# shayneobrien/generative-models

Measured on AMD Instinct MI355X. Metric: images/sec (28x28 MNIST) per D+G step, NSGAN bs=256, higher is better.
Workload: dtype f32; 1 GPU; NSGAN MNIST bs=256 fp32 per GPU (BASELINE.json configs[1]); 784-400-20 MLPs, N=50000 synthetic Bernoulli images, parity-mode RNG protocol, Adam 2e-4, D_steps=1; global_batch=256, parallelism=dp1, ranks_seen=1, gradient_exchange=none (1 rank), timing=one 2064-step timed region, cold_start_inclusive=False

## Files before the change

generative_models_amd/csrc/gm_gemm.hip:

```cpp
#include "gm_common.h"
#include "gm_head.h"
#include "gm_gather.h"
#include "gm_dvae.h"
#include "gm_ldsdma.h"

#include <cstdlib>
#include <type_traits>

typedef float f32x16 __attribute__((ext_vector_type(16)));

#ifdef GM_STAMPS
namespace gm_stamps {
constexpr int WAVES = 16, IDS = 40, HDR = 8, MAXB = 512, SLOT_WORDS = HDR + 2 * MAXB + WAVES * IDS * 2, SLOTS = 64;
static unsigned long long* host_buf = nullptr;
static int host_tile = 0, host_next = 0;
struct Ctx { unsigned long long* slot; int tile; };
__device__ __forceinline__ void rec(const Ctx& c, int tile, int id) {
    if (!c.slot || tile != c.tile || (threadIdx.x & 63)) return;
    __builtin_amdgcn_sched_barrier(0);
    unsigned long long* w = c.slot + HDR + 2 * MAXB + ((threadIdx.x >> 6) * IDS + id) * 2;
    w[0] = clock64(); w[1] = wall_clock64();
    __builtin_amdgcn_sched_barrier(0);
}
__device__ __forceinline__ void edge(const Ctx& c, bool exit_, int tile, int M, int N, int K, int mode) {
    if (!c.slot || threadIdx.x) return;
    const int blk = blockIdx.y * gridDim.x + blockIdx.x;
    if (blk < MAXB) c.slot[HDR + 2 * blk + (exit_ ? 1 : 0)] = wall_clock64();
    if (!exit_ && tile == 0) {
        c.slot[0] = 1; c.slot[2] = (unsigned long long)gridDim.x * gridDim.y; c.slot[3] = M; c.slot[4] = N; c.slot[5] = K;
        c.slot[6] = mode; c.slot[7] = blockDim.x;
    }
}
}
#define GM_STAMP(ctx, tile, id) gm_stamps::rec((ctx), (tile), (id))
#define GM_STAMP_EDGE(p, exit_, tile, mode) gm_stamps::edge((p).stamp, (exit_), (tile), (p).M, (p).N, (p).K, (mode))
#define GM_STAMP_AFTER(v) asm volatile("" ::"v"(v))
extern "C" int gm_stamps_set(unsigned long long* dev_buf, int probe_tile) {
    gm_stamps::host_buf = dev_buf; gm_stamps::host_tile = probe_tile; gm_stamps::host_next = 0;
    return 0;
}
extern "C" int gm_stamps_layout(int* out6) {
    out6[0] = gm_stamps::WAVES; out6[1] = gm_stamps::IDS; out6[2] = gm_stamps::HDR; out6[3] = gm_stamps::SLOT_WORDS;
    out6[4] = gm_stamps::SLOTS; out6[5] = gm_stamps::MAXB;
    return 0;
}
#else
#define GM_STAMP(slot, tile, id) do {} while (0)
#define GM_STAMP_EDGE(p, exit_, tile, mode) do {} while (0)
#define GM_STAMP_AFTER(v) do {} while (0)
#endif

namespace {

constexpr int TM = 32, TN = 32;

enum { MODE_FWD = 0, MODE_DX = 1, MODE_DW = 2 };

struct GemmP {
// ... 157 lines not shown
        }
    } else if (MODE == MODE_DX) {
        if (p.add) {
            const float4 a = ld4(p.add + (int64_t)m * p.ldadd + n);
            v.x += p.add_scale * a.x; v.y += p.add_scale * a.y; v.z += p.add_scale * a.z; v.w += p.add_scale * a.w;
        }
        if (p.epi == GM_ACT_RELU) {
            const float4 y = ld4(p.aux + (int64_t)m * p.ldaux + n);
            v.x = (y.x > 0.f) ? v.x : 0.f; v.y = (y.y > 0.f) ? v.y : 0.f; v.z = (y.z > 0.f) ? v.z : 0.f; v.w = (y.w > 0.f) ? v.w : 0.f;
        } else if (p.epi == GM_ACT_SIGMOID) {
            const float4 y = ld4(p.aux + (int64_t)m * p.ldaux + n);
            v.x = v.x * (y.x * (1.f - y.x)); v.y = v.y * (y.y * (1.f - y.y));
            v.z = v.z * (y.z * (1.f - y.z)); v.w = v.w * (y.w * (1.f - y.w));
        }
        float* cp = p.C + (int64_t)m * p.ldc + n;
        if (p.accumulate) { const float4 c = ld4(cp); v.x = c.x + v.x; v.y = c.y + v.y; v.z = c.z + v.z; v.w = c.w + v.w; }
        st4(cp, v);
    } else {
        const int64_t o = (int64_t)m * p.ldc + n;
        if (p.accumulate) { const float4 c = ld4(p.C + o); v.x += c.x; v.y += c.y; v.z += c.z; v.w += c.w; }
        st4(p.C + o, v);
        if (p.adam.enabled) {
            const int64_t si = gm_slot_index(p.adam.sched_slot);
            const float step_size = p.adam.sched[2 * si], bc2_sqrt = p.adam.sched[2 * si + 1];
            float4 P = ld4(p.adam.pW + o), M = ld4(p.adam.mW + o), V = ld4(p.adam.vW + o);
            adam_update(P.x, v.x, M.x, V.x, step_size, bc2_sqrt, p.adam.omb1, p.adam.b2, p.adam.omb2, p.adam.eps, p.adam.wd, p.adam.clamp);
            adam_update(P.y, v.y, M.y, V.y, step_size, bc2_sqrt, p.adam.omb1, p.adam.b2, p.adam.omb2, p.adam.eps, p.adam.wd, p.adam.clamp);
            adam_update(P.z, v.z, M.z, V.z, step_size, bc2_sqrt, p.adam.omb1, p.adam.b2, p.adam.omb2, p.adam.eps, p.adam.wd, p.adam.clamp);
            adam_update(P.w, v.w, M.w, V.w, step_size, bc2_sqrt, p.adam.omb1, p.adam.b2, p.adam.omb2, p.adam.eps, p.adam.wd, p.adam.clamp);
            st4(p.adam.pW + o, P); st4(p.adam.mW + o, M); st4(p.adam.vW + o, V);
        }
    }
}

template <int MODE>
__device__ __forceinline__ void store_group(const GemmP& p, float4 v, int m, int n, int ncap) {
    const int nreal = (MODE == MODE_DW) ? p.n_real : p.N;
    if (n + 3 < nreal && n + 3 < ncap) { store4<MODE>(p, v, m, n); return; }
    if (n < p.N && n < ncap) store_element<MODE>(p, v.x, m, n);
    if (n + 1 < p.N && n + 1 < ncap) store_element<MODE>(p, v.y, m, n + 1);
    if (n + 2 < p.N && n + 2 < ncap) store_element<MODE>(p, v.z, m, n + 2);
    if (n + 3 < p.N && n + 3 < ncap) store_element<MODE>(p, v.w, m, n + 3);
}

__device__ __forceinline__ int red_idx(int w, int row, int col) {
    return (w * 32 + row) * 32 + (col ^ ((((row >> 2) ^ row) & 1) << 4));
}

__device__ __forceinline__ int red_idx_sx(int w, int row, int col, int flip) {
    return (w * 32 + row) * 32 + (col ^ flip);
}

constexpr int KEEP_LD = 68;
template <int MODE, int WAVES, int ROWS = 32, bool LBL = false, int SXD = 0>
__device__ __forceinline__ void reduce_and_store(const GemmP& p, const float* red, int t, int m0,
                                                 int n0, int ncap = 0x7fffffff, int rcap = 32,
                                                 float* kept = nullptr, int srow0 = 0) {
    if (MODE == MODE_FWD && p.hd_part) {
#pragma unroll
        for (int e = 0; e < 1024 / (WAVES * 64); ++e) {
            const int row = (t >> 5) + e * (WAVES * 2), col = t & 31;
            const bool live = !(ROWS < 32 && row >= ROWS) && row < rcap;
            float v = 0.f;
            if (live) {
#pragma unroll
                for (int ww = 0; ww < WAVES; ++ww) v += red[red_idx(ww, row, col)];
            }
            const int m = m0 + row, n = n0 + col;
            const bool ok = live && m < p.M && n < p.N && n < ncap;
            float pv = 0.f;
            if (ok) {
                const float w = p.hd_w2[n];
                const float y = fwd_value(p, v, n);
                p.C[(int64_t)m * p.ldc + n] = y;
                pv = y * w;
                if (m == 0 && p.hd_snap) {
                    p.hd_snap[n] = w;
                    if (n == 0) p.hd_snap[p.N] = p.hd_b2[0];
                }
            }
#pragma unroll
            for (int o = 16; o > 0; o >>= 1) pv += __shfl_xor(pv, o, 64);
            if (col == 0 && live && m < p.M) p.hd_part[(int64_t)m * p.hd_ldp + (n0 >> 5)] = pv;
        }
        return;
    }
    if (MODE == MODE_FWD && p.sq_part) {
#pragma unroll
        for (int e = 0; e < 1024 / (WAVES * 64); ++e) {
            const int row = (t >> 5) + e * (WAVES * 2), col = t & 31;
            const bool live = !(ROWS < 32 && row >= ROWS) && row < rcap;
            float v = 0.f;
            if (live) {
#pragma unroll
                for (int ww = 0; ww < WAVES; ++ww) v += red[red_idx(ww, row, col)];
            }
            const int m = m0 + row, n = n0 + col;
            const bool ok = live && m < p.M && n < p.N && n < ncap;
            float pv = 0.f;
            if (ok) {
                const float r = fwd_value(p, v, n);
                p.C[(int64_t)m * p.ldc + n] = r;
                const float d = p.sq_x[(int64_t)m * p.sq_ldx + n] - r;
                pv = d * d;
                const float go = -(2.f * d);
                p.sq_dA[(int64_t)m * p.sq_lda + n] = (go * (1.f - r)) * r;
            }
#pragma unroll
            for (int o = 16; o > 0; o >>= 1) pv += __shfl_xor(pv, o, 64);
            if (col == 0 && live && m < p.M) p.sq_part[(int64_t)m * p.sq_ldp + (n0 >> 5)] = pv;
        }
        return;
    }
#pragma unroll
    for (int e = 0; e < 1024 / (WAVES * 64); ++e) {
        const int row = (t >> 5) + e * (WAVES * 2), col = t & 31;
        if ((ROWS < 32 && row >= ROWS) || row >= rcap) continue;
        float v = 0.f;
#pragma unroll
        for (int ww = 0; ww < WAVES; ++ww)
            v += red[SXD > 0 ? red_idx_sx(ww, row, col, ((srow0 + row) / (SXD > 0 ? SXD : 1)) & 1) : red_idx(ww, row, col)];
        const int m = m0 + row, n = n0 + col;
        if (m >= p.M || n >= p.N || n >= ncap) continue;
        store_element<MODE, LBL>(p, v, m, n, kept ? kept + row * KEEP_LD + col : nullptr);
    }
}

__device__ __forceinline__ float4 keep4(bool ok, float4 v) {
    return make_float4(ok ? v.x : 0.f, ok ? v.y : 0.f, ok ? v.z : 0.f, ok ? v.w : 0.f);
}

template <int NMFMA, int NDSR, int NVMEM, int NDSW>
__device__ __forceinline__ void lds_stage_schedule() {
    constexpr int NMEM = NDSR + NVMEM + NDSW;
    int done = 0;
#pragma unroll
    for (int q = 0; q < NMFMA; ++q) {
        __builtin_amdgcn_sched_group_barrier(0x008, 1, 0);
        const int upto = (NMEM * (q + 1) + NMFMA - 1) / NMFMA;
#pragma unroll
        for (int i = 0; i < 8; ++i) {
            if (done < upto) {
                if (done < NDSR) __builtin_amdgcn_sched_group_barrier(0x100, 1, 0);
                else if (done < NDSR + NVMEM) __builtin_amdgcn_sched_group_barrier(0x020, 1, 0);
                else __builtin_amdgcn_sched_group_barrier(0x200, 1, 0);
                ++done;
            }
        }
    }
}

template <int MODE, int BM, int BN, int WTM, int WTN, int WK, int KU>
struct LdsCfg {
    static constexpr int WM = BM / WTM, WN = BN / WTN, NW = WM * WN * WK, NT = 64 * NW, BK = 8 * WK * KU;
    static constexpr int TI = WTM / 32, TJ = WTN / 32;
    static constexpr bool B_KC = (MODE == MODE_FWD);
    static constexpr int LDK = BK + 4, LDXB = BN + 4;
    static constexpr int A_SZ = BM * LDK;
    static constexpr int B_SZ = B_KC ? BN * LDK : BK * LDXB;
    static constexpr int STAGE = A_SZ + B_SZ;
    static constexpr int NBUF = 3;
    static constexpr int RED = WK * BM * BN;
    static constexpr int FLOATS = (NBUF * STAGE > RED) ? NBUF * STAGE : RED;
};

template <int MODE, int BM, int BN, int WTM, int WTN, int WK, int KU, int PD, int NS>
__global__ __launch_bounds__(64 * (BM / WTM) * (BN / WTN) * WK) void gemm_lds_kernel(GemmP p) {
    using C = LdsCfg<MODE, BM, BN, WTM, WTN, WK, KU>;
    constexpr int NT = C::NT, BK = C::BK, LDK = C::LDK, LDXB = C::LDXB, TI = C::TI, TJ = C::TJ;
// ... 599 lines not shown
    constexpr bool XMAP_A = MODE == MODE_DW && XV, XMAP_B = MODE != MODE_FWD && XV;
    const int ia = XMAP_A ? sigma16(i16) : i16, ib = XMAP_B ? sigma16(i16) : i16;
    if constexpr (FOLD == 1 && SX) {
#pragma unroll
        for (int mi = 0; mi < MI; ++mi) fws[mi] = p.fold_w2[min(xla + mi, p.M - 1)];
    } else if constexpr (FOLD == 1) {
#pragma unroll
        for (int mi = 0; mi < MI; ++mi)
            fw[mi] = *reinterpret_cast<const float4*>(
                p.fold_w2 + min(m0 + 16 * mi + 4 * xq_ld, p.M - 4));
    }
    auto load_a = [&](int c, int mi) -> FragA {
        const int kb = 16 * c + 4 * g4, x0 = m0 + 16 * mi;
        if constexpr (SXA) return raw_xs<MI>(A, p.lda, xla, p.M, kb + mi, p.K);
        else {
            if (MODE == MODE_DW) {
                if (XV) return raw_xc4_16(A, p.lda, x0, p.M, c, p.K, lane);
                return raw_xc(A, p.lda, x0 + i16, p.M, kb, p.K);
            }
            return raw_kc<VEC>(A, p.lda, x0 + i16, p.M, kb, p.K);
        }
    };
    auto load_b = [&](int c, int ni) -> FragB {
        const int kb = 16 * c + 4 * g4, x0 = n0 + 16 * ni;
        if constexpr (SX) return raw_xs<NI>(B, p.ldb, xlb, b_cols, kb + ni, p.K);
        else {
            if (MODE == MODE_FWD) return raw_kc<VEC>(B, p.ldb, x0 + i16, p.N, kb, p.K);
            if (XV) return raw_xc4_16(B, p.ldb, x0, b_cols, c, p.K, lane);
            return raw_xc(B, p.ldb, x0 + i16, b_cols, kb, p.K);
        }
    };
    auto fix_a = [&](float4 v, int c, int mi, float4 wk) -> float4 {
        const int kb = 16 * c + 4 * g4, x = m0 + 16 * mi + ia;
        if constexpr (FOLD == 1)
            v = fold_dh4(v, sds[min(16 * c + 4 * g4 + xe_ld, p.K - 1)], fw[mi]);
        if constexpr (FOLD == 2) v = fold_dh4(v, fds[mi], wk);
        if (MODE == MODE_DW)
            return fix_xc(XV ? lane48_transpose(v, lane) : v, x, p.M, kb, p.K, -1);
        return fix_kc(v, x, p.M, kb, p.K);
    };
    auto fix_b = [&](float4 v, int c, int ni) -> float4 {
        const int kb = 16 * c + 4 * g4, x = n0 + 16 * ni + ib;
        if (MODE == MODE_FWD) return fix_kc(v, x, p.N, kb, p.K);
        return fix_xc(XV ? lane48_transpose(v, lane) : v, x, b_cols, kb, p.K, ones_col, OF ? p.ones_from : 0);
    };

    f32x4 acc[MI][NI];
#pragma unroll
    for (int mi = 0; mi < MI; ++mi)
#pragma unroll
        for (int ni = 0; ni < NI; ++ni) acc[mi][ni] = f32x4{0.f, 0.f, 0.f, 0.f};

    const int nq = (nchunks - w + WAVES - 1) / WAVES;
    auto consume = [&](const FragA (&ra)[NA], const FragB (&rb)[NB], float4 wk, int q) {
        const int cq = w + q * WAVES;
        if constexpr (SX) {
            float fa[4][MI], fb[4][NI];
            if constexpr (!SXA) {
#pragma unroll
                for (int mi = 0; mi < MI; ++mi) {
                    const float4 v = fix_a(ra[mi], cq, mi, wk);
                    fa[0][mi] = v.x; fa[1][mi] = v.y; fa[2][mi] = v.z; fa[3][mi] = v.w;
                }
            }
#pragma unroll
            for (int t4 = 0; t4 < 4; ++t4) {
                const int k = 16 * cq + 4 * g4 + t4;
                const bool kin = k < p.K;
                if constexpr (SXA) {
                    float ds = 0.f;
                    if constexpr (FOLD == 1) ds = sds[min(k, p.K - 1)];
                    fix_xs<MI, FOLD == 1>(ra[t4], fa[t4], xla, p.M, kin, -1, 0.f, ds, fws);
                }
                float one = 1.f;
                if constexpr (OF) one = (k >= p.ones_from) ? 1.f : 0.f;
                fix_xs<NI, false>(rb[t4], fb[t4], xlb, b_cols, kin, ones_col, one, 0.f, nullptr);
            }
            GM_STAMP_AFTER(fa[3][MI - 1]); GM_STAMP_AFTER(fb[3][NI - 1]);
            if (q < 4) GM_STAMP(st_slot, st_tile, 1 + 2 * q);
#pragma unroll
            for (int mi = 0; mi < MI; ++mi)
#pragma unroll
                for (int ni = 0; ni < NI; ++ni) {
                    f32x4 c4 = acc[mi][ni];
#pragma unroll
                    for (int t4 = 0; t4 < 4; ++t4)
                        c4 = __builtin_amdgcn_mfma_f32_16x16x4f32(fa[t4][mi], fb[t4][ni], c4, 0, 0, 0);
                    acc[mi][ni] = c4;
                }
        } else {
        float4 fa[MI], fb[NI];
#pragma unroll
        for (int mi = 0; mi < MI; ++mi) fa[mi] = fix_a(ra[mi], cq, mi, wk);
#pragma unroll
        for (int ni = 0; ni < NI; ++ni) fb[ni] = fix_b(rb[ni], cq, ni);
        GM_STAMP_AFTER(fa[MI - 1].x); GM_STAMP_AFTER(fb[NI - 1].x);
        if (q < 4) GM_STAMP(st_slot, st_tile, 1 + 2 * q);
#pragma unroll
        for (int mi = 0; mi < MI; ++mi)
#pragma unroll
            for (int ni = 0; ni < NI; ++ni) {
                f32x4 c4 = acc[mi][ni];
                c4 = __builtin_amdgcn_mfma_f32_16x16x4f32(fa[mi].x, fb[ni].x, c4, 0, 0, 0);
                c4 = __builtin_amdgcn_mfma_f32_16x16x4f32(fa[mi].y, fb[ni].y, c4, 0, 0, 0);
                c4 = __builtin_amdgcn_mfma_f32_16x16x4f32(fa[mi].z, fb[ni].z, c4, 0, 0, 0);
                c4 = __builtin_amdgcn_mfma_f32_16x16x4f32(fa[mi].w, fb[ni].w, c4, 0, 0, 0);
                acc[mi][ni] = c4;
// ... 141 lines not shown
    }
    GM_STAMP(st_slot, st_tile, 9);
    if constexpr (SX) {
        if constexpr (MODE == MODE_DW && MI * NI > 4) {
            if (p.vec_epi) {
                dw_reduce_onepass<MI, NI, false, false, true>(p, red, acc, m0, n0, false);
                GM_STAMP(st_slot, st_tile, 12);
                GM_STAMP_EDGE(p, true, st_tile, MODE);
                return;
            }
        }
        sx_block_reduce<MODE, MI, NI, SXA>(p, red, acc, m0, n0, kept);
        GM_STAMP(st_slot, st_tile, 12);
        GM_STAMP_EDGE(p, true, st_tile, MODE);
        return;
    }
    if constexpr (MODE == MODE_DW && WAVES == 16 && MI * NI > 4) {
        if (p.vec_epi) {
            dw_reduce_onepass<MI, NI, false, XMAP_A>(p, red, acc, m0, n0, false);
            GM_STAMP(st_slot, st_tile, 12);
            GM_STAMP_EDGE(p, true, st_tile, MODE);
            return;
        }
    }
#pragma unroll
    for (int bm = 0; bm < (MI + 1) / 2; ++bm)
#pragma unroll
        for (int bn = 0; bn < (NI + 1) / 2; ++bn) {
            if (bm + bn > 0) __syncthreads();
#pragma unroll
            for (int rgi = 0; rgi < 4; ++rgi) {
                const int row = XMAP_A ? sigma16(g4 * 4 + rgi) : g4 * 4 + rgi;
                red[red_idx(w, row, ib)] = acc[2 * bm][2 * bn][rgi];
                if (2 * bn + 1 < NI) red[red_idx(w, row, 16 + ib)] = acc[2 * bm][(2 * bn + 1 < NI) ? 2 * bn + 1 : 0][rgi];
                if (2 * bm + 1 < MI) {
                    constexpr int MIX = MI > 1 ? MI - 1 : 0;
                    const int mu = (2 * bm + 1 < MI) ? 2 * bm + 1 : MIX;
                    red[red_idx(w, 16 + row, ib)] = acc[mu][2 * bn][rgi];
                    if (2 * bn + 1 < NI)
                        red[red_idx(w, 16 + row, 16 + ib)] = acc[mu][(2 * bn + 1 < NI) ? 2 * bn + 1 : 0][rgi];
                }
            }
            __syncthreads();
            if (bm + bn == 0) GM_STAMP(st_slot, st_tile, 10);
            reduce_and_store<MODE, WAVES, (MI > 1 ? 32 : 16), LBL>(p, red, t, m0 + 32 * bm, n0 + 32 * bn,
                                                              (2 * bn + 1 < NI) ? 0x7fffffff : n0 + 32 * bn + 16,
                                                              (2 * bm + 1 < MI) ? 32 : 16,
                                                              kept ? kept + 32 * bm * KEEP_LD + 32 * bn : nullptr);
        }
    GM_STAMP(st_slot, st_tile, 12);
    GM_STAMP_EDGE(p, true, st_tile, MODE);
}

template <int MODE, bool VEC, int WAVES, int G, bool XV, int MI, int NI, bool DMA = false, bool SL = false>
__global__ __launch_bounds__(WAVES * 64) void gemm16_kernel(GemmP p) {
    __shared__ __attribute__((aligned(16))) float red[(WAVES == 16) ? RedSize<MODE, DMA, MI, NI>::value : WAVES * 32 * 32];
    gemm16_body<MODE, VEC, WAVES, G, XV, MI, NI, false, 0, DMA, false, false, SL>(p, red, blockIdx.x, blockIdx.y, nullptr, nullptr,
                                                                                  (int)gridDim.x);
}

template <bool VEC, int MI, int NI>
__global__ __launch_bounds__(1024) void gemm16_fwd_label_kernel(GemmP p) {
    __shared__ __attribute__((aligned(16))) float red[RedSize<MODE_FWD, false, MI, NI>::value];
    gemm16_body<MODE_FWD, VEC, 16, 1, false, MI, NI, false, 0, false, false, false, false, true>(p, red, blockIdx.x, blockIdx.y,
                                                                                                nullptr, nullptr, (int)gridDim.x);
}

template <int MODE, bool VEC, int G, bool XV, int MI, int NI, bool OF = false, bool FOLDED = false, bool DMA = false,
          bool TP = false, bool PK = false>
__device__ __forceinline__ void gemm16_with_head(const GemmP& p, const HeadBwdP& hp, int hrows,
                                                 int hblocks) {
    __shared__ __attribute__((aligned(16))) float red[RedSize<MODE, DMA, MI, NI>::value];
    __shared__ float sds[FOLDED ? FOLD_MAX_ROWS : 1];
    constexpr int FOLD = FOLDED ? (MODE == MODE_DW ? 1 : 2) : 0;
    if ((int)blockIdx.y < hrows) {
        const int bid = blockIdx.y * gridDim.x + blockIdx.x;
        if (bid < hblocks) head_bwd_body<TP>(hp, bid, sds);
        return;
    }
    gemm16_body<MODE, VEC, 16, G, XV, MI, NI, OF, FOLD, DMA, TP, PK, false>(p, red, blockIdx.x, blockIdx.y - hrows, sds, &hp.fold,
                                                                            (int)gridDim.x);
}

template <bool VEC, int G, bool XV, int MI, int NI, bool OF = false, bool FOLDED = false, bool DMA = false>
__global__ __launch_bounds__(1024) void gemm16_dw_head_kernel(GemmP p, HeadBwdP hp, int hrows,
                                                              int hblocks) {
    gemm16_with_head<MODE_DW, VEC, G, XV, MI, NI, OF, FOLDED, DMA>(p, hp, hrows, hblocks);
}

__global__ __launch_bounds__(1024) void gemm16_fwd_bits_kernel(GemmP p) {
    __shared__ __attribute__((aligned(16))) float red[RedSize<MODE_FWD, false, 2, 2>::value];
    gemm16_body<MODE_FWD, true, 16, 1, false, 2, 2, false, 0, false, false, true, false>(p, red, blockIdx.x, blockIdx.y);
}
__global__ __launch_bounds__(1024) void gemm16_dw_head_bits_kernel(GemmP p, HeadBwdP hp, int hrows, int hblocks) {
    gemm16_with_head<MODE_DW, false, 1, true, 2, 3, false, true, false, false, true>(p, hp, hrows, hblocks);
}

template <int MI, int NI>
__global__ __launch_bounds__(1024) void gemm16_dw_head_tp_kernel(GemmP p, HeadBwdP hp, int hrows, int hblocks) {
    gemm16_with_head<MODE_DW, false, 1, true, MI, NI, false, true, false, true>(p, hp, hrows, hblocks);
}

template <int G, int MI, int NI, bool FOLDED = false>
__global__ __launch_bounds__(1024) void gemm16_dx_head_kernel(GemmP p, HeadBwdP hp, int hrows,
                                                              int hblocks) {
    gemm16_with_head<MODE_DX, true, G, true, MI, NI, false, FOLDED>(p, hp, hrows, hblocks);
}

inline bool aligned16(const void* p) { return (reinterpret_cast<uintptr_t>(p) & 15) == 0; }
// ... 209 lines not shown
        }
    }
}

template <int MI, int NI>
__global__ __launch_bounds__(1024) void gemm16_dw_pair_l1_kernel(GemmP pa, GemmP pb, int na, int tna, L1RideP r) {
    __shared__ __attribute__((aligned(16))) float red[RedSize<MODE_DW, false, MI, NI>::value];
    __shared__ __attribute__((aligned(16))) float kept[16 * KEEP_LD];
    static_assert(NI <= 4 && 16 * NI <= KEEP_LD, "one 16-row tile of [W1 | b1] in `kept`");
    const int id = blockIdx.x;
    if (id < na) {
        gemm16_body<MODE_DW, false, 16, 1, true, MI, NI, false, 0, false, false, false, false>(pa, red, id % tna, id / tna);
        return;
    }
    const int by = id - na;
    gemm16_body<MODE_DW, false, 16, 1, true, 1, NI, false, 0, false, false, false, true>(pb, red, 0, by, nullptr, nullptr, 0,
                                                                                        kept);
    __syncthreads();
    l1_ride_fwd(r, kept, 16 * by, pb.M, pb.n_real);
}

template <int MODE>
int vec_epi_ok(const GemmP& p) {
    if (!aligned16(p.C) || p.ldc % 4 != 0) return 0;
    if (MODE == MODE_FWD) {
        if (p.bias && !aligned16(p.bias)) return 0;
        if (p.ip_out && !(aligned16(p.ip_out) && aligned16(p.ip_x) && p.ip_ldo % 4 == 0 && p.ip_ldx % 4 == 0)) return 0;
    } else if (MODE == MODE_DX) {
        if (p.epi != GM_ACT_ID && !(aligned16(p.aux) && p.ldaux % 4 == 0)) return 0;
        if (p.add && !(aligned16(p.add) && p.ldadd % 4 == 0)) return 0;
    } else {
        if (p.adam.enabled && !(aligned16(p.adam.pW) && aligned16(p.adam.mW) && aligned16(p.adam.vW))) return 0;
    }
    return 1;
}

struct Rider {
    const HeadBwdP* head = nullptr;
    const GatherP* gather = nullptr;
    const CorruptP* corrupt = nullptr;
    const GemmP* pair = nullptr;
    bool pair_xvec = false;
    const gm_fin2* fin = nullptr;
    const L1RideP* l1 = nullptr;
};

inline void launch_gather_alone(hipStream_t s, const Rider& r) {
    const GatherP& gp = *r.gather;
    if (r.corrupt)
        hipLaunchKernelGGL(gather_rows_corrupt_kernel, dim3(gm_gather_blocks(gp, 4)), dim3(256), 0, s, gp, *r.corrupt);
    else
        hipLaunchKernelGGL(gather_rows_kernel, dim3(gm_gather_blocks(gp, 4)), dim3(256), 0, s, gp);
}

enum { T22 = 0, T24, T42, T12, T23, T32 };
inline int tile_mi(int t) { return t == T42 ? 4 : t == T32 ? 3 : t == T12 ? 1 : 2; }
inline int tile_ni(int t) { return t == T24 ? 4 : t == T23 ? 3 : 2; }

template <int MODE>
int pick_tile(const GemmP& p) {
    const int tm = (p.M + TM - 1) / TM, tn = (p.N + TN - 1) / TN;
    int t = T22;
    if (tm * tn > 256 && (p.K + 15) / 16 >= 32) t = (tn >= tm) ? T24 : T42;
    else if (tm * tn <= 128 && p.M > 16) t = T12;
    if (MODE == MODE_DW) {
        if (t == T24 && tm * ((p.N + 47) / 48) <= 256) t = T23;
        else if (t == T42 && tn * ((p.M + 47) / 48) <= 256) t = T32;
        else if (t == T22 && tm * tn > 256) {
            if (tn >= tm && tm * ((p.N + 47) / 48) <= 256) t = T23;
            else if (tn < tm && tn * ((p.M + 47) / 48) <= 256) t = T32;
        }
    }
    if (MODE == MODE_FWD && t == T42 && !p.hd_part && !p.sq_part && tn * ((p.M + 47) / 48) <= 256) t = T32;
    return t;
}

#define GM_TILE_SWITCH(tile, dma, LAUNCH)                                           \
    do {                                                                            \
        switch (tile) {                                                             \
        case T24: LAUNCH(2, 4, false); break;                                       \
        case T42: LAUNCH(4, 2, false); break;                                       \
        case T12: LAUNCH(1, 2, false); break;                                       \
        case T23: if (dma) LAUNCH(2, 3, true); else LAUNCH(2, 3, false); break;     \
        case T32: if (dma) LAUNCH(3, 2, true); else LAUNCH(3, 2, false); break;     \
        default: LAUNCH(2, 2, false); break;                                        \
        }                                                                           \
    } while (0)

template <int MODE>
int launch(hipStream_t s, const GemmP& p_in, bool vec, bool xvec = false, const Rider& rider = Rider()) {
    const HeadBwdP* head = rider.head;
    const bool folded = head && head->fold.enabled;
    GemmP p = p_in;
    p.vec_epi = vec_epi_ok<MODE>(p);
#ifdef GM_STAMPS
    p.stamp.slot = gm_stamps::host_buf ? gm_stamps::host_buf + (size_t)(gm_stamps::host_next++ % gm_stamps::SLOTS) * gm_stamps::SLOT_WORDS
                                       : nullptr;
    p.stamp.tile = gm_stamps::host_tile;
#endif
    const bool xv = xvec && MODE != MODE_FWD;
    const bool slots = has_slot(p.a_slot) || has_slot(p.b_slot);
    if (slots && (folded || p.pk_bits)) {
        gm_set_error("ring slots on the operands of a folded-head / bit-packed launch are not supported");
        return GM_EINVAL;
    }
    const bool ride_head = head && !slots;
// ... 168 lines not shown
                r2.l1 = nullptr;
                const int rc = launch<MODE_DW>(s, p_in, vec, xvec, r2);
                if (rc) return rc;
                const L1RideP& l = *rider.l1;
                GemmP f{};
                f.A = l.z; f.B = pb.adam.pW; f.C = l.H; f.M = l.rows; f.N = pb.M; f.K = pb.n_real;
                f.lda = l.ldz; f.ldb = pb.ldc; f.ldc = l.ldh; f.bias = pb.adam.pb; f.epi = GM_ACT_RELU;
                f.a_slot = l.z_slot; f.b_slot = gm_slot{};
                const bool fvec = aligned16(l.z) && aligned16(pb.adam.pW) && (l.ldz % 4 == 0) && (f.K % 4 == 0) &&
                                  (pb.ldc % 4 == 0) && (l.z_slot.stride % 4 == 0);
                return launch<MODE_FWD>(s, f, fvec);
            }
            if (pairable) {
                const bool dma = p.dma && dma_ok(pb, true);
                p.dma = pb.dma = dma;
                const int tna = (int)grid.x, na = (int)(grid.x * grid.y);
                if (l1_rides) {
                    const dim3 lgrid(na + (pb.M + 15) / 16);
#define GM_LL1(MI_, NI_, D_) hipLaunchKernelGGL((gemm16_dw_pair_l1_kernel<MI_, NI_>), lgrid, dim3(1024), 0, s, p, pb, na, tna, *rider.l1)
                    GM_TILE_SWITCH(tile, false, GM_LL1);
#undef GM_LL1
                    GM_LAUNCH_RET();
                }
                const int tnb = (pb.N + 16 * ni - 1) / (16 * ni), tmb = (pb.M + 16 * mi - 1) / (16 * mi);
                const dim3 pgrid(na + tnb * tmb);
                const bool sl_b = has_slot(pb.a_slot) || has_slot(pb.b_slot);
#define GM_LP2(K_, GRID_, MI_, NI_, D_, ...)                                                                              \
    do {                                                                                                                  \
        if (slots) hipLaunchKernelGGL((K_<1, true, MI_, NI_, D_, true, true>), GRID_, dim3(1024), 0, s, __VA_ARGS__);     \
        else if (sl_b) hipLaunchKernelGGL((K_<1, true, MI_, NI_, D_, false, true>), GRID_, dim3(1024), 0, s, __VA_ARGS__); \
        else hipLaunchKernelGGL((K_<1, true, MI_, NI_, D_, false, false>), GRID_, dim3(1024), 0, s, __VA_ARGS__);         \
    } while (0)
#define GM_LP(MI_, NI_, D_) GM_LP2(gemm16_dw_pair_kernel, pgrid, MI_, NI_, D_, p, pb, na, tna, tnb)
#define GM_LPF(MI_, NI_, D_) GM_LP2(gemm16_dw_pair_fin_kernel, dim3(pgrid.x + 1), MI_, NI_, D_, p, pb, na, tna, tnb, *rider.fin)
                if (rider.fin) GM_TILE_SWITCH(tile, dma, GM_LPF);
                else GM_TILE_SWITCH(tile, dma, GM_LP);
#undef GM_LP2
#undef GM_LPF
#undef GM_LP
                GM_LAUNCH_RET();
            }
            Rider none;
            int rc = launch<MODE_DW>(s, p_in, vec, xvec, none);
            if (rc) return rc;
            rc = launch<MODE_DW>(s, pb, false, rider.pair_xvec, none);
            if (rc || !rider.fin) return rc;
            const gm_fin2& f = *rider.fin;
            return gm_sum_finalize2_tick(s, f.pa, f.na, f.sa, f.oa, f.slot_a, f.pb, f.nb, f.sb, f.ob, f.slot_b, f.tick);
        }
    }
    if (MODE == MODE_DX && slots) { gm_set_error("ring slots: forward and weight-gradient operands only"); return GM_EINVAL; }
#define GM_L16K(V, X, MI_, NI_, D_)                                                                                          \
    do {                                                                                                                     \
        if (MODE != MODE_DX && slots)                                                                                        \
            hipLaunchKernelGGL((gemm16_kernel<MODE, V, 16, 1, X, MI_, NI_, (MODE == MODE_DW && (X) && (D_)), MODE != MODE_DX>), grid, dim3(1024), 0, s, p); \
        else                                                                                                                 \
            hipLaunchKernelGGL((gemm16_kernel<MODE, V, 16, 1, X, MI_, NI_, (MODE == MODE_DW && (X) && (D_)), false>), grid, dim3(1024), 0, s, p); \
    } while (0)
#define GM_L16_tt(MI_, NI_, D_) GM_L16K(true, true, MI_, NI_, D_)
#define GM_L16_tf(MI_, NI_, D_) GM_L16K(true, false, MI_, NI_, D_)
#define GM_L16_ft(MI_, NI_, D_) GM_L16K(false, true, MI_, NI_, D_)
#define GM_L16_ff(MI_, NI_, D_) GM_L16K(false, false, MI_, NI_, D_)
    if (xv) { if (vec) GM_TILE_SWITCH(tile, p.dma, GM_L16_tt); else GM_TILE_SWITCH(tile, p.dma, GM_L16_ft); }
    else    { if (vec) GM_TILE_SWITCH(tile, false, GM_L16_tf); else GM_TILE_SWITCH(tile, false, GM_L16_ff); }
#undef GM_L16_ff
#undef GM_L16_ft
#undef GM_L16_tf
#undef GM_L16_tt
#undef GM_L16K
    GM_LAUNCH_RET();
}

inline gm_slot no_slot() { gm_slot z; z.ctr = nullptr; z.mul = 0; z.add = 0; z.ring = 0; z.stride = 0; return z; }

}



static int gather_from_args(const gm_gather_args& a, bool forward, GatherP* g, CorruptP* c, const CorruptP** rider_c,
                            const float** gout) {
    GM_CHECK_ARG(!a.data != !a.bits);
    GM_CHECK_ARG(!a.out != !a.out_bits);
    GM_CHECK_ARG(!a.out_bits || (a.bits && forward));
    GM_CHECK_ARG(!a.corrupt == !a.out_c);
    GM_CHECK_ARG(!a.corrupt || forward);
    int rc;
    if (a.data) rc = gm_gather_fill(a.data, a.n_rows, a.idx, a.idx_slot, a.out, a.ld_out, a.B, a.row_elems, g);
    else if (a.out) rc = gm_gather_fill_bits(a.bits, a.words_per_row, a.n_rows, a.idx, a.idx_slot, a.out, a.ld_out, a.B,
                                             a.row_elems, g);
    else rc = gm_gather_fill_bits_packed(a.bits, a.words_per_row, a.n_rows, a.idx, a.idx_slot, a.out_bits, a.B, g);
    if (rc) return rc;
    *rider_c = nullptr;
    if (a.corrupt) {
        rc = gm_gather_corrupt_fill(a.corrupt, a.out_c, g, c);
        if (rc) return rc;
        *rider_c = c;
    }
    *gout = a.out ? a.out : reinterpret_cast<const float*>(a.out_bits);
    return 0;
}

static bool slot_is_zero(const gm_slot& s) { return !s.ctr && !s.mul && !s.add && !s.ring && !s.stride; }

static int fwd_label_launch(hipStream_t s, const GemmP& p, bool vec);

static int fwd_impl(void* stream, const gm_fwd_args* args) {
// ... 22 lines not shown
    GatherP g{};
    CorruptP c{};
    if (interp) {
        GM_CHECK_ARG(a.ip_eps && a.ip_x && a.ip_out && a.ip_rows > 0 && a.ip_rows <= a.M && a.ip_ldx >= a.N &&
                     a.ip_ldo >= a.N);
        p.ip_eps = a.ip_eps; p.ip_slot = a.ip_slot; p.ip_x = a.ip_x; p.ip_ldx = a.ip_ldx;
        p.ip_out = a.ip_out; p.ip_ldo = a.ip_ldo; p.ip_rows = a.ip_rows;
    } else if (head) {
        GM_CHECK_ARG(a.hd_w2 && a.hd_b2 && a.hd_part && a.hd_snap && a.hd_ldp >= (a.N + 31) / 32 && a.hd_ldp % 4 == 0);
        GM_CHECK_ARG(a.hd_part != a.Y && a.hd_snap != a.Y && (const float*)a.hd_part != a.X &&
                     (const float*)a.hd_snap != a.X);
        p.hd_w2 = a.hd_w2; p.hd_b2 = a.hd_b2; p.hd_part = a.hd_part; p.hd_ldp = a.hd_ldp; p.hd_snap = a.hd_snap;
        if (a.xbits) {
            GM_CHECK_ARG(a.xbits_rows > 0 && a.xbits_rows <= a.M && a.xbits_rows % 32 == 0 &&
                         a.xbits_wpr * 32 >= a.K && a.K % 4 == 0);
            GM_CHECK_ARG((const void*)a.xbits != (const void*)a.Y && (const void*)a.xbits != (const void*)a.hd_part);
            p.pk_bits = a.xbits; p.pk_wpr = a.xbits_wpr; p.pk_rows = a.xbits_rows;
        }
    } else if (sqerr) {
        GM_CHECK_ARG(a.act == GM_ACT_SIGMOID);
        GM_CHECK_ARG(a.sq_target && a.sq_dA && a.sq_part && a.sq_ldt >= a.N && a.sq_lda >= a.N &&
                     a.sq_ldp >= (a.N + 31) / 32);
        GM_CHECK_ARG(a.sq_dA != a.Y && a.sq_part != a.Y && a.sq_part != a.sq_dA && (const float*)a.sq_dA != a.X &&
                     (const float*)a.sq_part != a.X && (const float*)a.Y != a.sq_target &&
                     (const float*)a.sq_dA != a.sq_target);
        p.sq_x = a.sq_target; p.sq_ldx = a.sq_ldt; p.sq_dA = a.sq_dA; p.sq_lda = a.sq_lda; p.sq_part = a.sq_part;
        p.sq_ldp = a.sq_ldp;
    } else if (label) {
        GM_CHECK_ARG(a.lb_E && a.lb.labels && a.lb_C > 0 && a.lb_C <= 32);
        p.lb = a.lb; p.lb_E = a.lb_E; p.lb_C = a.lb_C;
        return fwd_label_launch((hipStream_t)stream, p, vec);
    } else if (a.gather) {
        const float* gout = nullptr;
        const int rc = gather_from_args(*a.gather, true, &g, &c, &r.corrupt, &gout);
        if (rc) return rc;
        GM_CHECK_ARG(gout != a.Y && gout != a.X);
        GM_CHECK_ARG(!r.corrupt || (c.out_c != a.Y && (const float*)c.out_c != a.X));
        r.gather = &g;
    }
    return launch<MODE_FWD>((hipStream_t)stream, p, vec, false, r);
}

static int fwd_label_launch(hipStream_t s, const GemmP& p, bool vec) {
    const int tile = pick_tile<MODE_FWD>(p);
    const dim3 grid((p.N + 16 * tile_ni(tile) - 1) / (16 * tile_ni(tile)), (p.M + 16 * tile_mi(tile) - 1) / (16 * tile_mi(tile)));
#define GM_LBL(MI_, NI_, D_)                                                                                \
    do {                                                                                                    \
        if (vec) hipLaunchKernelGGL((gemm16_fwd_label_kernel<true, MI_, NI_>), grid, dim3(1024), 0, s, p);  \
        else hipLaunchKernelGGL((gemm16_fwd_label_kernel<false, MI_, NI_>), grid, dim3(1024), 0, s, p);     \
    } while (0)
    GM_TILE_SWITCH(tile, false, GM_LBL);
#undef GM_LBL
    GM_LAUNCH_RET();
}

extern "C" int gm_linear_fwd(void* stream, const float* X, int64_t ldx, gm_slot x_slot, const float* W,
                             const float* bias, float* Y, int64_t ldy, int M, int K, int N, int act) {
    gm_fwd_args a{};
    a.X = X; a.ldx = ldx; a.x_slot = x_slot; a.W = W; a.bias = bias; a.Y = Y; a.ldy = ldy;
    a.M = M; a.K = K; a.N = N; a.act = act;
    return fwd_impl(stream, &a);
}

extern "C" int gm_linear_fwd_ex(void* stream, const gm_fwd_args* a) { return fwd_impl(stream, a); }

static int dx_impl(void* stream, const gm_dx_args* args) {
    GM_CHECK_ARG(args);
    const gm_dx_args& a = *args;
    GM_CHECK_ARG(a.dA && a.W && a.dX && a.M > 0 && a.K > 0 && a.N > 0 && a.lda >= a.N && a.ldx >= a.K);
    GM_CHECK_ARG(a.epi == GM_ACT_ID || (a.below && a.ld_below >= a.K));
    const bool reparam = a.rp_ml || a.rp_eps || a.rp_dml;
    if ((a.add != nullptr) + (a.head != nullptr) + reparam + (a.gather != nullptr) > 1) {
        gm_set_error("gm_dx_args: at most one of the add / head / reparam / gather blocks");
        return GM_EINVAL;
    }
    if (a.fold && !a.head) { gm_set_error("gm_dx_args: fold needs head"); return GM_EINVAL; }
    if (reparam && (a.below || a.ld_below || a.epi != GM_ACT_ID)) {
        gm_set_error("gm_dx_args: the reparameterisation epilogue takes no activation gradient");
        return GM_EINVAL;
    }
    GemmP p{};
    p.A = a.dA; p.B = a.W; p.C = a.dX; p.M = a.M; p.N = a.K; p.K = a.N;
    p.lda = a.lda; p.ldb = a.K; p.ldc = a.ldx; p.aux = a.below; p.ldaux = a.ld_below; p.epi = a.epi;
    p.a_slot = no_slot(); p.b_slot = no_slot();
    Rider r;
    HeadBwdP hp{};
    GatherP g{};
    if (a.add) {
        GM_CHECK_ARG(a.ldadd >= a.K);
        p.add = a.add; p.ldadd = a.ldadd; p.add_scale = a.add_scale;
    } else if (a.head && a.fold) {
        GM_CHECK_ARG(a.head->gen_mode && a.head->H == a.dA && a.head->B == a.M && a.head->Hd == a.N);
        GM_CHECK_ARG((const float*)a.dX != a.dA && a.dX != a.fold->S && a.dX != a.fold->dS && a.dX != a.fold->rowloss);
        const int rc = gm_head_from_args(*a.head, &hp, a.fold);
        if (rc) return rc;
        p.fold_w2 = a.fold->snap;
        r.head = &hp;
    } else if (a.head) {
        GM_CHECK_ARG((const float*)a.dX != a.head->H && (const float*)a.dX != a.head->dS &&
                     (const float*)a.dX != a.head->rowloss && a.dX != a.head->dH);
        const int rc = gm_head_from_args(*a.head, &hp);
        if (rc) return rc;
        r.head = &hp;
    } else if (reparam) {
        GM_CHECK_ARG(a.rp_ml && a.rp_eps && a.rp_dml && a.rp_ldml >= 2 * a.K && a.rp_ldd >= 2 * a.K &&
                     a.rp_dml != a.dX && (const float*)a.rp_dml != a.rp_ml && (const float*)a.rp_dml != a.dA);
// ... 145 lines not shown
```

generative_models_amd/ops.py:

```python
import ctypes

import numpy as np
import torch

from . import _lib
from ._lib import ACT, LOSS, NO_SLOT, Slot, slot


def stream_ptr():
    return torch.cuda.current_stream().cuda_stream


def _chk(t, name):
    if not (t.is_cuda and t.dtype == torch.float32):
        raise _lib.GMError("%s must be a float32 device tensor (got %s on %s)" %
                           (name, t.dtype, t.device))
    return t


def _ld(t):
    if t.dim() == 1:
        return 1
    if t.stride(1) != 1:
        raise _lib.GMError("inner dimension must be contiguous")
# ... 222 lines not shown
    assert fin["done"].dtype == torch.int32 and fin["done"].numel() >= 1
    f.done = fin["done"].data_ptr()
    t = _lib.DwTail()
    t.fin = ctypes.pointer(f)
    _dw_ex(a, b, t, stream)


def _head_args(head, betas=(0.9, 0.999), eps=1e-8):
    hl, ha, H = head["lin"], head.get("adam"), head["H"]
    gen = bool(head.get("gen_mode", False))
    a = _lib.HeadBwdArgs()
    a.H, a.ldh, a.dS = H.data_ptr(), _ld(H), _ptr(head.get("dS"))
    a.w2, a.b2, a.rowloss = hl.W.data_ptr(), hl.b.data_ptr(), _ptr(head.get("rowloss"))
    a.dH, a.lddh = None, 0
    if not gen:
        a.gw2, a.gb2 = hl.gW.data_ptr(), hl.gb.data_ptr()
    a.loss_out, a.loss_slot = head["loss_out"].data_ptr(), head["loss_slot"]
    a.inv_b, a.gen_mode, a.B, a.Hd = head["inv_b"], 1 if gen else 0, head["B"], H.shape[1]
    a.with_adam = 1 if ha is not None else 0
    if ha is not None:
        a.mW, a.vW, a.mb, a.vb = hl.mW.data_ptr(), hl.vW.data_ptr(), hl.mb.data_ptr(), hl.vb.data_ptr()
        a.sched, a.sched_slot = ha["sched"].data_ptr(), ha["sched_slot"]
        a.clamp = ha.get("clamp", 0.0)
    a.beta1, a.beta2, a.eps, a.weight_decay = betas[0], betas[1], eps, 0.0
    a.tick, a.gw2_add, a.gb2_add = _ptr(head.get("tick")), _ptr(head.get("gw2_add")), _ptr(head.get("gb2_add"))
    pen = head.get("pen")
    if pen is not None:
        a.pen_s, a.pen_h, a.pen_ldh = pen["s"].data_ptr(), pen["h"].data_ptr(), _ld(pen["h"])
        a.pen_t, a.pen_ldt, a.pen_rows = pen["t"].data_ptr(), _ld(pen["t"]), pen["t"].shape[0]
    return a


def linear_fwd_sqerr(x, W, b, y, target, dA, part, M=None, stream=None):
    a = _fwd_args(x, W, b, y, "sigmoid", M)
    assert part.dim() == 2 and part.shape[0] >= a.M and part.shape[1] >= (a.N + 31) // 32
    a.sq_target, a.sq_ldt = _chk(target, "target").data_ptr(), _ld(target)
    a.sq_dA, a.sq_lda = _chk(dA, "dA").data_ptr(), _ld(dA)
    a.sq_part, a.sq_ldp = part.data_ptr(), part.shape[1]
    _fwd_ex(a, stream)
    return y


def linear_bwd_dx_reparam(dA, W, dZ, ml, eps, dml, M=None, eps_slot=NO_SLOT, stream=None):
    a = _dx_args(dA, W, dZ, M=M)
    a.rp_ml, a.rp_ldml, a.rp_eps, a.rp_slot = ml.data_ptr(), _ld(ml), eps.data_ptr(), eps_slot
    a.rp_dml, a.rp_ldd = dml.data_ptr(), _ld(dml)
    _dx_ex(a, stream)
    return dZ


def lds_min_m():
    import os
    return 1024


class HeadFold:

    def __init__(self, rows, hidden, device):
        self.nparts = (hidden + 31) // 32
        assert self.nparts <= 16, "folded head: hidden layers up to 512 wide"
        self.part = torch.zeros(rows, _al4(self.nparts), device=device)
        self.snap = torch.zeros(_al4(hidden + 1), device=device)
        self.hidden = hidden

    def args(self, variant, out_act, hyper=(), pen=None, S=None, dS=None, rowloss=None):
        a = _lib.HeadFoldArgs()
        a.part, a.ldp, a.nparts, a.snap = self.part.data_ptr(), self.part.shape[1], self.nparts, self.snap.data_ptr()
        a.variant = LOSS[variant] if not isinstance(variant, int) else variant
        a.out_act = _act(out_act)
        hy = tuple(hyper)
        assert len(hy) <= 8
        for i, h in enumerate(hy):
            a.hyper[i] = float(h)
        a.n_hyper = len(hy)
        a.pen, a.S, a.dS, a.rowloss = _ptr(pen), _ptr(S), _ptr(dS), _ptr(rowloss)
        return a


def _al4(n):
    return (n + 3) // 4 * 4


def linear_fwd_headpart(x, W, b, y, act, head_lin, fold, M=None, x_slot=NO_SLOT, stream=None, xbits=None):
    a = _fwd_args(x, W, b, y, act, M, x_slot)
    assert fold.hidden == a.N and fold.part.shape[0] >= a.M
    a.hd_w2, a.hd_b2, a.hd_snap = head_lin.W.data_ptr(), head_lin.b.data_ptr(), fold.snap.data_ptr()
    a.hd_part, a.hd_ldp = fold.part.data_ptr(), fold.part.shape[1]
    if xbits is not None:
        a.xbits, a.xbits_wpr, a.xbits_rows = xbits[0].data_ptr(), xbits[1], xbits[2]
    _fwd_ex(a, stream)
    return y


def linear_bwd_dx_head_fold(H, W, dX, head, fold_args, below=None, epi="id", M=None, stream=None):
    a = _dx_args(H, W, dX, below, epi, M)
    h = _head_args(head)
    a.head, a.fold = ctypes.pointer(h), ctypes.pointer(fold_args)
    _dx_ex(a, stream)
    return dX


def linear_bwd_dw_adam_head_fold(H, X, lin, adam, head, fold_args, M=None, x_slot=NO_SLOT,
                                 betas=(0.9, 0.999), eps=1e-8, weight_decay=0.0, stream=None, xbits=None):
    a = _dw_adam_args(H, X, lin, adam, M, x_slot, betas, eps, weight_decay)
    h = _head_args(head, betas, eps)
    a.head, a.fold = ctypes.pointer(h), ctypes.pointer(fold_args)
# ... 303 lines not shown
```

Baseline: 4.327 million images/sec.

## Add 8-wave two-stream forward GEMM kernel replacing 16-wave split-K path

Adds a forward GEMM variant that runs 8 hardware waves, each carrying two interleaved K-chunk streams with separate accumulators and register double-buffered global loads, in place of 16 waves. The LDS split-K reduction keeps 16 partial images and reduces them with the 8-wave thread count. It is the default for vectorized non-transposed forward tiles without ring slots, and a runtime switch can force the old 16-wave path. The aim is to halve block size and overlap loads with MFMA inside each wave, at the cost of more registers per wave and less wave-level parallelism.

```diff
diff --git a/generative_models_amd/csrc/gm_gemm.hip b/generative_models_amd/csrc/gm_gemm.hip
--- a/generative_models_amd/csrc/gm_gemm.hip
+++ b/generative_models_amd/csrc/gm_gemm.hip
@@ -4,6 +4,7 @@
 #include "gm_dvae.h"
 #include "gm_ldsdma.h"
 
+#include <atomic>
 #include <cstdlib>
 #include <type_traits>
 
@@ -267,14 +268,14 @@
 }
 
 constexpr int KEEP_LD = 68;
-template <int MODE, int WAVES, int ROWS = 32, bool LBL = false, int SXD = 0>
+template <int MODE, int WAVES, int ROWS = 32, bool LBL = false, int SXD = 0, int HW = WAVES>
 __device__ __forceinline__ void reduce_and_store(const GemmP& p, const float* red, int t, int m0,
                                                  int n0, int ncap = 0x7fffffff, int rcap = 32,
                                                  float* kept = nullptr, int srow0 = 0) {
     if (MODE == MODE_FWD && p.hd_part) {
 #pragma unroll
-        for (int e = 0; e < 1024 / (WAVES * 64); ++e) {
-            const int row = (t >> 5) + e * (WAVES * 2), col = t & 31;
+        for (int e = 0; e < 1024 / (HW * 64); ++e) {
+            const int row = (t >> 5) + e * (HW * 2), col = t & 31;
             const bool live = !(ROWS < 32 && row >= ROWS) && row < rcap;
             float v = 0.f;
             if (live) {
@@ -302,8 +303,8 @@
     }
     if (MODE == MODE_FWD && p.sq_part) {
 #pragma unroll
-        for (int e = 0; e < 1024 / (WAVES * 64); ++e) {
-            const int row = (t >> 5) + e * (WAVES * 2), col = t & 31;
+        for (int e = 0; e < 1024 / (HW * 64); ++e) {
+            const int row = (t >> 5) + e * (HW * 2), col = t & 31;
             const bool live = !(ROWS < 32 && row >= ROWS) && row < rcap;
             float v = 0.f;
             if (live) {
@@ -328,8 +329,8 @@
         return;
     }
 #pragma unroll
-    for (int e = 0; e < 1024 / (WAVES * 64); ++e) {
-        const int row = (t >> 5) + e * (WAVES * 2), col = t & 31;
+    for (int e = 0; e < 1024 / (HW * 64); ++e) {
+        const int row = (t >> 5) + e * (HW * 2), col = t & 31;
         if ((ROWS < 32 && row >= ROWS) || row >= rcap) continue;
         float v = 0.f;
 #pragma unroll
@@ -1035,7 +1036,7 @@
         for (int ni = 0; ni < NI; ++ni) acc[mi][ni] = f32x4{0.f, 0.f, 0.f, 0.f};
 
     const int nq = (nchunks - w + WAVES - 1) / WAVES;
-    auto consume = [&](const FragA (&ra)[NA], const FragB (&rb)[NB], float4 wk, int q) {
+    auto consume =[&](const FragA (&ra)[NA], const FragB (&rb)[NB], float4 wk, int q) {
         const int cq = w + q * WAVES;
         if constexpr (SX) {
             float fa[4][MI], fb[4][NI];
@@ -1283,9 +1284,124 @@
     GM_STAMP_EDGE(p, true, st_tile, MODE);
 }
 
+template <int MI, int NI, bool LBL = false>
+__device__ __forceinline__ void gemm16_fwd_streams2(const GemmP& p, float* red, int bx, int by) {
+    constexpr int STREAMS = 16, HW = 8;
+    const int t = threadIdx.x, lane = t & 63;
+    const int w = __builtin_amdgcn_readfirstlane(t >> 6);
+    const int i16 = lane & 15, g4 = lane >> 4;
+    const int m0 = by * (16 * MI), n0 = bx * (16 * NI);
+    const float* A = p.A;
+    const float* B = p.B;
+    const int nchunks = (p.K + 15) >> 4;
+    const int nqa = (nchunks - w + STREAMS - 1) / STREAMS, nqb = (nchunks - w - HW + STREAMS - 1) / STREAMS;
+
+    f32x4 acc_a[MI][NI], acc_b[MI][NI];
+#pragma unroll
+    for (int mi = 0; mi < MI; ++mi)
+#pragma unroll
+        for (int ni = 0; ni < NI; ++ni) acc_a[mi][ni] = acc_b[mi][ni] = f32x4{0.f, 0.f, 0.f, 0.f};
+
+    auto load_kc = [&](const float* __restrict__ P, int64_t ld, int x, int X, int c) -> f32x4 {
+        return *reinterpret_cast<const f32x4*>(P + (int64_t)min(x, X - 1) * ld + min(16 * c + 4 * g4, p.K - 4));
+    };
+#define GM_S2_LOAD(ra, rb, c)                                                                            \
+    _Pragma("unroll") for (int mi = 0; mi < MI; ++mi) ra[mi] = load_kc(A, p.lda, m0 + 16 * mi + i16, p.M, (c)); \
+    _Pragma("unroll") for (int ni = 0; ni < NI; ++ni) rb[ni] = load_kc(B, p.ldb, n0 + 16 * ni + i16, p.N, (c));
+    auto consume = [&](const f32x4 (&ra)[MI], const f32x4 (&rb)[NI], f32x4 (&acc)[MI][NI], int c) {
+        const int kb = 16 * c + 4 * g4;
+        float4 fa[MI], fb[NI];
+#pragma unroll
+        for (int mi = 0; mi < MI; ++mi)
+            fa[mi] = fix_kc(make_float4(ra[mi][0], ra[mi][1], ra[mi][2], ra[mi][3]), m0 + 16 * mi + i16, p.M, kb, p.K);
+#pragma unroll
+        for (int ni = 0; ni < NI; ++ni)
+            fb[ni] = fix_kc(make_float4(rb[ni][0], rb[ni][1], rb[ni][2], rb[ni][3]), n0 + 16 * ni + i16, p.N, kb, p.K);
+#pragma unroll
+        for (int mi = 0; mi < MI; ++mi)
+#pragma unroll
+            for (int ni = 0; ni < NI; ++ni) {
+                f32x4 c4 = acc[mi][ni];
+                c4 = __builtin_amdgcn_mfma_f32_16x16x4f32(fa[mi].x, fb[ni].x, c4, 0, 0, 0);
+                c4 = __builtin_amdgcn_mfma_f32_16x16x4f32(fa[mi].y, fb[ni].y, c4, 0, 0, 0);
+                c4 = __builtin_amdgcn_mfma_f32_16x16x4f32(fa[mi].z, fb[ni].z, c4, 0, 0, 0);
+                c4 = __builtin_amdgcn_mfma_f32_16x16x4f32(fa[mi].w, fb[ni].w, c4, 0, 0, 0);
+                acc[mi][ni] = c4;
+            }
+    };
+    auto done = [&](f32x4 (&acc)[MI][NI]) {
+        if constexpr (MI == 2)
+            asm volatile("" : "+v"(acc[0][0]), "+v"(acc[0][1]), "+v"(acc[1][0]), "+v"(acc[1][1]) : : "memory");
+        else
+            asm volatile("" : "+v"(acc[0][0]), "+v"(acc[0][1]) : : "memory");
+    };
+    auto take = [&](f32x4 (&ra)[MI], f32x4 (&rb)[NI]) {
+        if constexpr (MI == 2) asm volatile("" : "+v"(ra[0]), "+v"(ra[1]), "+v"(rb[0]), "+v"(rb[1]) : : "memory");
+        else asm volatile("" : "+v"(ra[0]), "+v"(rb[0]), "+v"(rb[1]) : : "memory");
+    };
+
+    f32x4 xa[MI], xb[NI], ya[MI], yb[NI];
+    GM_S2_LOAD(xa, xb, w)
+    asm volatile("" : : : "memory");
+    GM_S2_LOAD(ya, yb, w + HW)
+    int q = 0;
+    for (; q + 1 < nqb; ++q) {
+        take(xa, xb);
+        consume(xa, xb, acc_a, w + q * STREAMS);
+        done(acc_a);
+        GM_S2_LOAD(xa, xb, w + (q + 1) * STREAMS)
+        take(ya, yb);
+        consume(ya, yb, acc_b, w + HW + q * STREAMS);
+        done(acc_b);
+        GM_S2_LOAD(ya, yb, w + HW + (q + 1) * STREAMS)
+    }
+    if (nqb > 0) {
+        take(xa, xb);
+        consume(xa, xb, acc_a, w + q * STREAMS);
+        done(acc_a);
+        if (nqa > nqb) {
+            GM_S2_LOAD(xa, xb, w + (q + 1) * STREAMS)
+            take(ya, yb);
+            consume(ya, yb, acc_b, w + HW + q * STREAMS);
+            done(acc_b);
+            take(xa, xb);
+            consume(xa, xb, acc_a, w + (q + 1) * STREAMS);
+        } else {
+            take(ya, yb);
+            consume(ya, yb, acc_b, w + HW + q * STREAMS);
+        }
+    } else if (nqa > 0) {
+        take(xa, xb);
+        consume(xa, xb, acc_a, w);
+    }
+#undef GM_S2_LOAD
+
+#pragma unroll
+    for (int s = 0; s < 2; ++s) {
+        const int img = w + s * HW;
+#pragma unroll
+        for (int rgi = 0; rgi < 4; ++rgi) {
+            const int row = g4 * 4 + rgi;
+#pragma unroll
+            for (int mi = 0; mi < MI; ++mi)
+#pragma unroll
+                for (int ni = 0; ni < NI; ++ni)
+                    red[red_idx(img, 16 * mi + row, 16 * ni + i16)] = s ? acc_b[mi][ni][rgi] : acc_a[mi][ni][rgi];
+        }
+    }
+    __syncthreads();
+    reduce_and_store<MODE_FWD, STREAMS, (MI > 1 ? 32 : 16), LBL, 0, HW>(p, red, t, m0, n0);
+}
+
 template <int MODE, bool VEC, int WAVES, int G, bool XV, int MI, int NI, bool DMA = false, bool SL = false>
 __global__ __launch_bounds__(WAVES * 64) void gemm16_kernel(GemmP p) {
-    __shared__ __attribute__((aligned(16))) float red[(WAVES == 16) ? RedSize<MODE, DMA, MI, NI>::value : WAVES * 32 * 32];
+    __shared__ __attribute__((aligned(16))) float red[(WAVES == 16) ? RedSize<MODE, DMA, MI, NI>::value : 16 * 32 * 32];
+    if constexpr (WAVES == 8) {
+        static_assert(MODE == MODE_FWD && VEC && !XV && !DMA && !SL && MI <= 2 && NI == 2,
+                      "8 hardware waves: the two-stream forward only");
+        gemm16_fwd_streams2<MI, NI>(p, red, blockIdx.x, blockIdx.y);
+        return;
+    } else
     gemm16_body<MODE, VEC, WAVES, G, XV, MI, NI, false, 0, DMA, false, false, SL>(p, red, blockIdx.x, blockIdx.y, nullptr, nullptr,
                                                                                   (int)gridDim.x);
 }
@@ -1601,6 +1717,8 @@
     else
         hipLaunchKernelGGL(gather_rows_kernel, dim3(gm_gather_blocks(gp, 4)), dim3(256), 0, s, gp);
 }
+
+std::atomic<int> g_force_waves16{0};
 
 enum { T22 = 0, T24, T42, T12, T23, T32 };
 inline int tile_mi(int t) { return t == T42 ? 4 : t == T32 ? 3 : t == T12 ? 1 : 2; }
@@ -1875,6 +1993,12 @@
     if (MODE == MODE_DX && slots) { gm_set_error("ring slots: forward and weight-gradient operands only"); return GM_EINVAL; }
 #define GM_L16K(V, X, MI_, NI_, D_)                                                                                          \
     do {                                                                                                                     \
+        if constexpr (MODE == MODE_FWD && (V) && !(X) && (MI_) <= 2 && (NI_) == 2) {                                         \
+            if (!slots && !g_force_waves16.load(std::memory_order_relaxed)) {                      \
+                hipLaunchKernelGGL((gemm16_kernel<MODE_FWD, true, 8, 1, false, MI_, NI_, false, false>), grid, dim3(512), 0, s, p); \
+                break;                                                                                                       \
+            }                                                                                                                \
+        }                                                                                                                    \
         if (MODE != MODE_DX && slots)                                                                                        \
             hipLaunchKernelGGL((gemm16_kernel<MODE, V, 16, 1, X, MI_, NI_, (MODE == MODE_DW && (X) && (D_)), MODE != MODE_DX>), grid, dim3(1024), 0, s, p); \
         else                                                                                                                 \
@@ -2003,6 +2127,11 @@
     GM_TILE_SWITCH(tile, false, GM_LBL);
 #undef GM_LBL
     GM_LAUNCH_RET();
+}
+
+extern "C" int gm_gemm_force_waves16(int on) {
+    if (on < 0) return g_force_waves16.load(std::memory_order_relaxed);
+    return g_force_waves16.exchange(on ? 1 : 0, std::memory_order_relaxed);
 }
 
 extern "C" int gm_linear_fwd(void* stream, const float* X, int64_t ldx, gm_slot x_slot, const float* W,
diff --git a/generative_models_amd/ops.py b/generative_models_amd/ops.py
--- a/generative_models_amd/ops.py
+++ b/generative_models_amd/ops.py
@@ -298,6 +298,12 @@
 def lds_min_m():
     import os
     return 1024
+
+
+def force_waves16(on=None):
+    fn = _lib.load().gm_gemm_force_waves16
+    fn.restype, fn.argtypes = ctypes.c_int, [ctypes.c_int]
+    return bool(fn(-1 if on is None else int(bool(on))))
 
 
 class HeadFold:
```

Result: slower. 4.201 million images/sec (-2.9%).
